# andabi/parallel-wavenet-vocoder

Measured on AMD Instinct MI355X. Metric: audio samples/sec, 4-flow IAF generation, higher is better.
Workload: dtype f32 via 3-term split-fp16 MFMA (fp32 accumulate, fp32 storage)

## Files before the change

### parallel-wavenet-vocoder_amd/csrc/pwv_layer_common.h

```cpp
#pragma once

#include "pwv_common.h"

namespace pwv {

constexpr int kA1 = 0;
constexpr int kA1Size = 4 * 16 * 64 * 4;
constexpr int kA2 = kA1 + kA1Size;
constexpr int kA2Size = 2 * 8 * 64 * 4;
constexpr int kBD = kA2 + kA2Size;
constexpr int kBDSize = 64;
constexpr int kLayerBase = kBD + kBDSize;
constexpr int kASSize = 4 * 8 * 64 * 4;
constexpr int kBSSize = 128;
constexpr int kCondC = 80;
constexpr int kACSize = 4 * (kCondC / 8) * 64 * 4;

constexpr int layer_floats(bool skip, bool cond) {
    return kLayerBase + (skip ? kASSize + kBSSize : 0) + (cond ? kACSize : 0);
}

constexpr int kHAS = 0;
constexpr int kHBS = kHAS + kASSize;
constexpr int kHA1 = kHBS + kBSSize;
constexpr int kHA1Size = 4 * 16 * 64 * 4;
constexpr int kHB1 = kHA1 + kHA1Size;
constexpr int kHW2 = kHB1 + 128;
constexpr int kMaxQ = 4;
constexpr int head_floats(int Q) { return kHW2 + 2 * Q * 64 + 4; }

struct LayerParams {
    const float* x_in[PWV_MAX_NETS];
    float* x_out[PWV_MAX_NETS];
    const float* packed[PWV_MAX_NETS];
    const float* proj[PWV_MAX_NETS];
    float* skip[PWV_MAX_NETS];
    const float* cond;
    int proj_row_stride;
    int G, N, T, dilation;
    int cond_hop, cond_offset, cond_frames;
    int skip_init;
    unsigned T_magic, T_shift;
    unsigned hop_magic, hop_shift;
    long long* trace;
    const float* x_first;
    const float* cfilt[PWV_MAX_NETS];
    const float* fold0[PWV_MAX_NETS];
    const float* packed_head[PWV_MAX_NETS];
    float* head_out[PWV_MAX_NETS];
    int head_q;
    float x_limit;
    int* range_flag;
};

struct StreamParams {
    const float* hist_rd;
    float* hist_wr;
    const int* slot_tab;
    long long block_stride;
    long long row_off[PWV_MAX_NETS];
    long long scalar_off;
};

inline void make_magic(unsigned d, unsigned& magic, unsigned& shift) {
    if (d <= 1) { magic = 0; shift = 0; return; }
    unsigned l = 0;
    while ((1ull << l) < d) ++l;
    const unsigned long long k = 31 + l;
    magic = (unsigned)(((1ull << k) + d - 1) / d);
    shift = l - 1;
}
__device__ __forceinline__ int fast_div(int n, unsigned magic, unsigned shift) {
    return magic ? (int)(__umulhi((unsigned)n, magic) >> shift) : n;
}

__device__ __forceinline__ void unit_rows(int unit, int lane, int rows, int N, int T, unsigned T_magic, unsigned T_shift,
                                          int& row, bool& valid, int& rc, int& n, int& t) {
    row = unit * 32 + (lane & 31);
    valid = row < rows;
    rc = valid ? row : rows - 1;
    if (T >= 32) {
        const int row0 = unit * 32;
        const int n0 = fast_div(row0, T_magic, T_shift);
        t = row0 - n0 * T + (lane & 31);
        n = n0;
        if (t >= T) { t -= T; n += 1; }
        if (!valid) { n = N - 1; t = T - 1; }
    } else {
        n = fast_div(rc, T_magic, T_shift);
        t = rc - n * T;
    }
}

constexpr int kVarlenRec = PWV_VARLEN_REC_INTS;
constexpr int kVarlenMinRows = 32;

__device__ __forceinline__ void unit_rows_varlen(const int* unit_map, int unit, int lane, int rows,
                                                 int& row, bool& valid, int& rc, int& fb, int& t) {
    typedef const __attribute__((address_space(4))) int* const_ints_t;
    row = unit * 32 + (lane & 31);
    valid = row < rows;
    rc = valid ? row : rows - 1;
    const int last = (rows - 1) >> 5;
    const const_ints_t rec = (const_ints_t)(unit_map + (size_t)(unit < last ? unit : last) * kVarlenRec);
    const int r0 = rec[1], f0 = rec[2], r1 = rec[3], f1 = rec[4];
    const bool second = rc >= r1;
    t = rc - (second ? r1 : r0);
    fb = second ? f1 : f0;
}

#ifdef PWV_TRACE
#define PWV_STAMP(slot)                                                                   \
    do {                                                                                  \
        if (p.trace && blockIdx.x < 2 && lane == 0 && tr_unit < 8)                        \
            p.trace[((blockIdx.x * 8 + wave) * 8 + tr_unit) * 16 + (slot)] = __builtin_amdgcn_s_memtime(); \
    } while (0)
#else
#define PWV_STAMP(slot) do {} while (0)
#endif

struct HeadParams {
    const float* in[PWV_MAX_NETS];
    const float* packed[PWV_MAX_NETS];
    float* out[PWV_MAX_NETS];
    int G, N, T, Q;
};

constexpr float kFScale = -2.8853900817779268f;
constexpr float kGScale = -1.4426950408889634f;
__device__ __forceinline__ float gate_act(float fs, float gs) {
#pragma clang fp contract(off)
    fs = __builtin_amdgcn_fmed3f(fs, -3.0e38f, 57.7f);
    gs = __builtin_amdgcn_fmed3f(gs, -3.0e38f, 57.7f);
    const float e1 = __builtin_amdgcn_exp2f(fs);
    const float e2 = __builtin_amdgcn_exp2f(gs);
    const float t = 1.f + e2;
    return (1.f - e1) * __builtin_amdgcn_rcpf(__builtin_fmaf(e1, t, t));
}

template <int N4, int THREADS>
__device__ __forceinline__ void fill_lds(float* lds, const float* __restrict__ packed, int tid) {
    constexpr int ITERS = (N4 + THREADS - 1) / THREADS;
    const f32x4* src = reinterpret_cast<const f32x4*>(packed);
    f32x4* dst = reinterpret_cast<f32x4*>(lds);
    f32x4 v[ITERS];
#pragma unroll
    for (int i = 0; i < ITERS; ++i) {
        const int idx = tid + i * THREADS;
        v[i] = src[idx < N4 ? idx : N4 - 1];
    }
#pragma unroll
    for (int i = 0; i < ITERS; ++i) {
        const int idx = tid + i * THREADS;
        if (idx < N4) dst[idx] = v[i];
    }
}

__host__ __device__ inline size_t tile32_floats(long long rows, int C) { return (size_t)((rows + 31) / 32) * 32 * C; }
__device__ __forceinline__ size_t tile_off(int row, int quad, int C) {
    return (size_t)(row >> 5) * (32 * C) + quad * 128 + (row & 31) * 4;
}
typedef unsigned u32x4 __attribute__((ext_vector_type(4)));
constexpr int kAuxWriteThrough = 16;
__device__ __forceinline__ __amdgpu_buffer_rsrc_t units_rsrc(const void* base, int u_begin, int u_end, int unit_bytes) {
    const unsigned long long a = (unsigned long long)base + (unsigned long long)u_begin * unit_bytes;
    const unsigned long long span = (unsigned long long)(u_end > u_begin ? u_end - u_begin : 0) * unit_bytes;
    const unsigned lo = __builtin_amdgcn_readfirstlane((unsigned)a), hi = __builtin_amdgcn_readfirstlane((unsigned)(a >> 32));
    const unsigned bytes = __builtin_amdgcn_readfirstlane((unsigned)(span > 0xffffffffull ? 0xffffffffull : span));
    return __builtin_amdgcn_make_buffer_rsrc((void*)(((unsigned long long)hi << 32) | lo), 0, bytes, 0x00020000);
}
__device__ __forceinline__ int units_off(int row, int quad, int C, int u_begin) {
    return (((row >> 5) - u_begin) * (32 * C) + quad * 128 + (row & 31) * 4) * 4;
}
template <typename V16>
__device__ __forceinline__ void store_wt(__amdgpu_buffer_rsrc_t r, int byte_off, V16 v) {
    static_assert(sizeof(V16) == 16, "store_wt moves 16 bytes");
    __builtin_amdgcn_raw_buffer_store_b128(__builtin_bit_cast(u32x4, v), r, byte_off, 0, kAuxWriteThrough);
}

typedef const __attribute__((address_space(1))) void* gptr_t;
typedef __attribute__((address_space(3))) void* lptr_t;
template <int N4, int WAVES>
__device__ __forceinline__ void fill_lds_dma(float* lds, const float* __restrict__ packed, int wave, int lane) {
    constexpr int CH = (N4 + 63) / 64;
#pragma unroll
    for (int i = 0; i < (CH + WAVES - 1) / WAVES; ++i) {
        const int c = wave + i * WAVES;
        if (c < CH && c * 64 + lane < N4)
            __builtin_amdgcn_global_load_lds((gptr_t)(packed + (size_t)(c * 64 + lane) * 4), (lptr_t)(lds + c * 256), 16, 0, 0);
    }
}

template <int NCH, int C>
__device__ __forceinline__ void load_tiled(const float* __restrict__ base, int row, int h, bool keep, float (&dst)[4 * NCH]) {
    const float* p0 = base + tile_off(row, h, C);
#pragma unroll
    for (int g = 0; g < NCH; ++g) {
        const f32x4 v = *reinterpret_cast<const f32x4*>(p0 + g * 256);
#pragma unroll
        for (int e = 0; e < 4; ++e) dst[4 * g + e] = keep ? v[e] : 0.f;
    }
}

template <int NCH>
__device__ __forceinline__ void load_row(const float* __restrict__ row, int h, bool keep, float (&dst)[4 * NCH]) {
#pragma unroll
    for (int g = 0; g < NCH; ++g) {
        const f32x4 v = *reinterpret_cast<const f32x4*>(row + 8 * g + 4 * h);
#pragma unroll
        for (int e = 0; e < 4; ++e) dst[4 * g + e] = keep ? v[e] : 0.f;
    }
}

template <int NCH>
__device__ __forceinline__ void load_contig(const float* __restrict__ p, float (&dst)[4 * NCH]) {
#pragma unroll
    for (int g = 0; g < NCH; ++g) {
        const f32x4 v = *reinterpret_cast<const f32x4*>(p + 4 * g);
#pragma unroll
        for (int e = 0; e < 4; ++e) dst[4 * g + e] = v[e];
    }
}


__device__ __forceinline__ f32x4 frag(const float* lds, int base, int it, int ngroups, int g, int lane) {
    return *reinterpret_cast<const f32x4*>(&lds[base + ((it * ngroups + g) * 64 + lane) * 4]);
}

template <int NG, int NIT, int IT0, int ITSTEP, int NACC, typename BF, typename EF, typename TF>
__device__ __forceinline__ void gemm_groups(const float* lds, int base, int lane, f32x16 (&acc)[NACC], f32x4 (&a)[4],
                                            BF&& bval, EF&& extra, TF&& tail) {
#pragma unroll
    for (int g = 0; g < NG; ++g) {
        f32x4 n[4] = {a[0], a[1], a[2], a[3]};
        if (g + 1 < NG) {
#pragma unroll
            for (int i = 0; i < NIT; ++i) n[i] = frag(lds, base, IT0 + i * ITSTEP, NG, g + 1, lane);
        } else {
            tail(n);
        }
        __builtin_amdgcn_sched_barrier(0);
#pragma unroll
        for (int e = 0; e < 4; ++e) {
            const float b = bval(g * 4 + e);
#pragma unroll
            for (int i = 0; i < NIT; ++i)
                acc[IT0 + i * ITSTEP] = __builtin_amdgcn_mfma_f32_32x32x2f32(a[i][e], b, acc[IT0 + i * ITSTEP], 0, 0, 0);
        }
        extra(g);
        __builtin_amdgcn_sched_barrier(0);
#pragma unroll
        for (int i = 0; i < 4; ++i) a[i] = n[i];
    }
}


int launch_stream_carry_ragged(const StreamParams& st, const int* tab, int n_carry, const int* cu_rows, int N, hipStream_t s);

int launch_layer_f16x3(const LayerParams& lp, bool skip, bool cond, bool gated, int per_net, hipStream_t s);
int launch_layer_f16x3_stream(const LayerParams& lp, const StreamParams& st, int per_net, hipStream_t s);
int launch_head_f16x3(const HeadParams& hp, bool from_gated, int grid, hipStream_t s);
int launch_pack_layer_f16x3(const float* filter, const float* gate, const float* dense, const float* dense_bias,
                            const float* skip, const float* skip_bias, const float* gc_filter, const float* gc_gate,
// ... 10 lines not shown
```

### parallel-wavenet-vocoder_amd/csrc/pwv_persist_exit.inc

```
    asm volatile("s_waitcnt vmcnt(0)" ::: "memory");
    if (!tail_done) {
        int old = 0;
        if (lane == 0) old = __hip_atomic_fetch_add(&ctl[4], 1, __ATOMIC_RELAXED, __HIP_MEMORY_SCOPE_WORKGROUP);
        if (__builtin_amdgcn_readfirstlane(old) == 7) {
            int done = 0;
            if (lane == 0) done = __hip_atomic_fetch_add(p.exited, 1, __ATOMIC_RELAXED, __HIP_MEMORY_SCOPE_AGENT);
            if (__builtin_amdgcn_readfirstlane(done) == p.active_wgs - 1) {
                for (int k = lane; k < p.G * p.nwg; k += 64) __hip_atomic_store(p.prog + (size_t)k * kProgStride, 0, __ATOMIC_RELAXED, __HIP_MEMORY_SCOPE_AGENT);
                if (SHORT) for (int k = lane; k < p.G * p.units; k += 64) __hip_atomic_store(p.uprog + (size_t)k * kUnitStride, 0, __ATOMIC_RELAXED, __HIP_MEMORY_SCOPE_AGENT);
                if (lane == 0) {
                    __hip_atomic_store(p.abort, 0, __ATOMIC_RELAXED, __HIP_MEMORY_SCOPE_AGENT);
                    __hip_atomic_store(p.exited, 0, __ATOMIC_RELAXED, __HIP_MEMORY_SCOPE_AGENT);
                }
            }
        }
    }
#ifdef PWV_PTRACE
    if (p.trace && lane == 0) {
        pt_acc[8] = __builtin_amdgcn_s_memtime();
        pt_acc[0] = pt_acc[8] - pt_start;
        long long* tr = p.trace + ((size_t)blockIdx.x * 8 + wave) * 24;
        for (int k = 0; k < 15; ++k) tr[k] = pt_acc[k];
        tr[16] = net; tr[17] = w; tr[18] = dead ? 1 : 0; tr[19] = __builtin_amdgcn_s_memrealtime(); tr[20] = pt_start_rt;
    }
#endif
```

### parallel-wavenet-vocoder_amd/csrc/pwv_persist_geometry.inc

```
    constexpr bool SHORT = MODE == 2;
    __shared__ __attribute__((aligned(16))) float lds[kLdsFloats];
    const int tid = threadIdx.x;
    const int lane = tid & 63;
    const int wave = __builtin_amdgcn_readfirstlane(tid >> 6);
    const int h = lane >> 5;

    int net, w;
    if (p.xcd_map) {
        const int x = blockIdx.x & 7, s = blockIdx.x >> 3;
        net = s % p.G;
        w = x * (p.nwg >> 3) + s / p.G;
    } else {
        net = blockIdx.x % p.G;
        w = blockIdx.x / p.G;
    }
    const int rows = p.N * p.T;
    auto rows_of = [&](int unit, int& row, bool& valid, int& rc, int& nn, int& t) {
        if constexpr (VARLEN) unit_rows_varlen(p.unit_map, unit, lane, rows, row, valid, rc, nn, t);
        else unit_rows(unit, lane, rows, p.N, p.T, p.T_magic, p.T_shift, row, valid, rc, nn, t);
    };
    auto p_base = [&](int nn) -> int {
        if constexpr (VARLEN) return nn;
        else return nn * p.cond_frames;
    };
    constexpr bool RAGGED = VARLEN && STREAM;
    auto unit_rec = [&](int unit, int& s0, int& r1) {
        typedef const __attribute__((address_space(4))) int* const_ints_t;
        const int last = (rows - 1) >> 5;
        const const_ints_t rec = (const_ints_t)(p.unit_map + (size_t)(unit < last ? unit : last) * kVarlenRec);
        s0 = rec[0];
        r1 = rec[3];
    };
    auto session_end = [&](int s0, int r1, bool second) -> int {
        return second ? p.cu_rows[s0 + 2] : r1;
    };
    (void)unit_rec;
    (void)session_end;
    const int u_begin = w * p.per_wg;
    const int u_end = u_begin + p.per_wg < p.units ? u_begin + p.per_wg : p.units;
    const int n = u_end - u_begin;
    if (n <= 0) return;
    const int L = p.n_layers;
    constexpr bool stat = SHORT;
    constexpr bool loader_mode = SHORT;
#ifdef PWV_PTRACE
    int pt_nev = 0;
#endif

    typedef __attribute__((address_space(3))) int* lds_ints_t;
    const lds_ints_t ctl = (lds_ints_t)(lds + kCtlF);
    typedef __attribute__((address_space(3))) volatile unsigned char* lds_bytes_t;
    const lds_bytes_t lb = (lds_bytes_t)lds;
    int* prog_n = p.prog + (size_t)net * p.nwg * kProgStride;
    int* uprog_n = p.uprog + (size_t)net * p.units * kUnitStride;
    const float* const proj_n = p.proj[net];
    const float* const packed_n = p.packed[net];
    const int v_dil = p.dil[lane & (kMaxPLayers - 1)];
    auto dil_of = [&](int j) -> int { return __builtin_amdgcn_readlane(v_dil, j); };
    auto dil_next = [&](int j) -> int { return j + 1 < L ? dil_of(j + 1) : (p.tail_q > 0 ? p.tail_dil : dil_of(j)); };

    for (int k = tid; k < (kLdsFloats - kCtlF); k += 512) ctl[k] = 0;
    __syncthreads();
    if (tid == 0) {
        lb[kSeenLB] = w > 0 ? 0 : 255;
        lb[kSeenRB] = w < p.last_wg ? 0 : 255;
        lb[kWreadyB] = 0;
        lb[kWreadyB + 1] = 1;
        lb[kTrueB] = 255;
    }
    auto fill_slot = [&](int slot, int layer, int first, int step) {
        const float* src = packed_n + (size_t)layer * p.packed_stride + lane * 4;
        float* dst = lds + slot * kSlot;
#pragma clang loop unroll(disable)
        for (int c = first; c < kSlot / 256; c += step)
            __builtin_amdgcn_global_load_lds((gptr_t)(src + c * 256), (lptr_t)(dst + c * 256), 16, 0, 0);
        if (first == 0 && lane < 16)
            __builtin_amdgcn_global_load_lds((gptr_t)(src + kSlotFull), (lptr_t)(lds + kBiasF + slot * 64), 16, 0, 0);
    };
    if (p.x_first && tid < 128) lds[kCfF + tid] = p.cfilt[net][tid];
    fill_slot(0, 0, wave, 8);
    if (L > 1) fill_slot(1, 1, wave, 8);
    __syncthreads();
    if (wave >= 4) __builtin_amdgcn_s_setprio(1);

    const __amdgpu_buffer_rsrc_t ring_rs = [&]() {
        const unsigned long long a = (unsigned long long)p.ring[net];
        const unsigned long long span = (unsigned long long)p.ring_stride * 8ull + (unsigned long long)p.units * 8192ull;
        const unsigned lo = __builtin_amdgcn_readfirstlane((unsigned)a), hi2 = __builtin_amdgcn_readfirstlane((unsigned)(a >> 32));
        return __builtin_amdgcn_make_buffer_rsrc((void*)(((unsigned long long)hi2 << 32) | lo), 0, __builtin_amdgcn_readfirstlane((unsigned)span), 0x00020000);
    }();
    const __amdgpu_buffer_rsrc_t proj_rs = [&]() {
        const unsigned long long a = (unsigned long long)proj_n;
        const unsigned lo = __builtin_amdgcn_readfirstlane((unsigned)a), hi2 = __builtin_amdgcn_readfirstlane((unsigned)(a >> 32));
        return __builtin_amdgcn_make_buffer_rsrc((void*)(((unsigned long long)hi2 << 32) | lo), 0, 0xFFFFFFFFu, 0x00020000);
    }();
    (void)proj_rs;
    const int slot_bytes = (int)(p.ring_stride * 4);
    int rot_pinned = 0;
    if constexpr (RAGGED) {
        rot_pinned = p.rot;
        asm volatile("" : "+s"(rot_pinned));
    }
    auto rot_of = [&]() -> int {
        if constexpr (RAGGED) return rot_pinned;
        else return p.rot;
    };
    auto in_soff = [&](int j) -> int { return ((j + 2 + rot_of()) % 3) * slot_bytes; };
    auto out_soff = [&](int j) -> int { return ((j + rot_of()) % 3) * slot_bytes; };
    auto toff = [&](int row) -> int { return ((row >> 5) * 2048 + h * 128 + (row & 31) * 4) * 4; };
    auto hist_lookback = [&](int jh, int d, int nn, int t, int unit, int rc, float (&xb)[32]) {
        if constexpr (STREAM) {
            if (!__all(t >= d)) {
                int sn = nn;
                if constexpr (RAGGED) {
                    int s0, r1, uu = unit;
                    asm volatile("" : "+s"(uu));
                    unit_rec(uu, s0, r1);
                    sn = s0 + (rc >= r1 ? 1 : 0);
                }
                if (t < d) {
                    const float* hr = p.hist_rd + (long long)p.slot_tab[2 * sn] * p.hist_block_stride + p.hist_off[net][jh] + tile_off(t, h, 64);
#pragma unroll
                    for (int g = 0; g < 8; ++g) {
                        const f32x4 v = *reinterpret_cast<const f32x4*>(hr + g * 256);
#pragma unroll
                        for (int e = 0; e < 4; ++e) xb[4 * g + e] = v[e];
                    }
                }
            }
        }
    };
    auto hist_store = [&](int jh, int d, int nn, int t, int unit, int rc, bool valid, const float (&xr)[32]) {
        if constexpr (RAGGED) {
            int s0, r1;
            unit_rec(unit, s0, r1);
            const bool second = rc >= r1;
            int k = rc + d - r1;
            if (__any(valid && (second || k >= 0))) {
                int lo = second ? 1 : 0;
                asm volatile("" : "+v"(lo));
                const int last = (rows - 1) >> 5;
                const int sn = p.unit_map[(size_t)(unit < last ? unit : last) * kVarlenRec] + lo;
                k = rc + d - p.cu_rows[sn + 1];
                if (valid && k >= 0) {
                    float* hw = p.hist_wr + (long long)p.slot_tab[2 * sn + 1] * p.hist_block_stride + p.hist_off[net][jh] + tile_off(k, h, 64);
#pragma unroll
                    for (int g = 0; g < 8; ++g) {
                        const f32x4 v = {xr[4 * g], xr[4 * g + 1], xr[4 * g + 2], xr[4 * g + 3]};
                        *reinterpret_cast<f32x4*>(hw + g * 256) = v;
                    }
                }
            }
        } else if constexpr (STREAM) {
            const int k = t + d - p.T;
            if (__any(valid && k >= 0)) {
                if (valid && k >= 0) {
                    float* hw = p.hist_wr + (long long)p.slot_tab[2 * nn + 1] * p.hist_block_stride + p.hist_off[net][jh] + tile_off(k, h, 64);
#pragma unroll
                    for (int g = 0; g < 8; ++g) {
                        const f32x4 v = {xr[4 * g], xr[4 * g + 1], xr[4 * g + 2], xr[4 * g + 3]};
                        *reinterpret_cast<f32x4*>(hw + g * 256) = v;
                    }
                }
            }
        }
    };

    auto load_x = [&](int j, int unit, float (&xb)[32], float (&xc)[32]) {
        int row, rc, nn, t;
        bool valid;
        rows_of(unit, row, valid, rc, nn, t);
        const int d = dil_of(j);
        const bool has_prev = t >= d;
        if (p.x_first && j == 0) {
            const float* x1 = p.x_first;
            xc[0] = x1[rc];
            xc[1] = t >= 1 ? x1[rc - (t >= 1 ? 1 : 0)] : 0.f;
            xb[0] = has_prev ? x1[rc - (has_prev ? d : 0)] : 0.f;
            xb[1] = t >= d + 1 ? x1[rc - (t >= d + 1 ? d + 1 : 0)] : 0.f;
#pragma unroll
            for (int k = 2; k < 32; ++k) xb[k] = xc[k] = 0.f;
            return;
        }
        const int so = in_soff(j);
        const int oc = toff(rc), ob = toff(has_prev ? rc - d : rc);
#pragma unroll
        for (int g = 0; g < 8; ++g) {
            const f32x4 v = __builtin_bit_cast(f32x4, __builtin_amdgcn_raw_buffer_load_b128(ring_rs, oc + g * 1024, so, 16));
#pragma unroll
            for (int e = 0; e < 4; ++e) xc[4 * g + e] = v[e];
        }
#pragma unroll
        for (int g = 0; g < 8; ++g) {
            const f32x4 v = __builtin_bit_cast(f32x4, __builtin_amdgcn_raw_buffer_load_b128(ring_rs, ob + g * 1024, so, 16));
#pragma unroll
            for (int e = 0; e < 4; ++e) xb[4 * g + e] = v[e];
        }
        if (!__all(has_prev)) {
#pragma unroll
            for (int k = 0; k < 32; ++k) xb[k] = has_prev ? xb[k] : 0.f;
        }
        hist_lookback(j, d, nn, t, unit, rc, xb);
    };

    auto load_xc = [&](int j, int unit, float (&xc)[32]) {
        int row, rc, nn, t;
        bool valid;
        rows_of(unit, row, valid, rc, nn, t);
        const int so = in_soff(j);
        const int oc = toff(rc);
#pragma unroll
        for (int g = 0; g < 8; ++g) {
            const f32x4 v = __builtin_bit_cast(f32x4, __builtin_amdgcn_raw_buffer_load_b128(ring_rs, oc + g * 1024, so, 16));
#pragma unroll
            for (int e = 0; e < 4; ++e) xc[4 * g + e] = v[e];
        }
    };
    auto load_xb = [&](int j, int unit, float (&xb)[32]) {
        int row, rc, nn, t;
        bool valid;
        rows_of(unit, row, valid, rc, nn, t);
        const int d = dil_of(j);
        const bool has_prev = t >= d;
        const int so = in_soff(j);
        const int ob = toff(has_prev ? rc - d : rc);
#pragma unroll
        for (int g = 0; g < 8; ++g) {
            const f32x4 v = __builtin_bit_cast(f32x4, __builtin_amdgcn_raw_buffer_load_b128(ring_rs, ob + g * 1024, so, 16));
#pragma unroll
            for (int e = 0; e < 4; ++e) xb[4 * g + e] = v[e];
        }
        hist_lookback(j, d, nn, t, unit, rc, xb);
    };
```

### parallel-wavenet-vocoder_amd/csrc/pwv_persist_tasks.inc

```
    if (u >= 0) {
        flush_owed();
        leave_layers(j);
        layer_vectors(j);
        if constexpr (SHORT) {
            load_xc(j, u, rxc);
        } else {
            const unsigned bad = eval(dep_addr(j, u));
            if (bad & kRawMask) wait_deps(j, u, kRawMask, j, 4);
            war_ok = (bad & kWarMask) == 0;
            if (!dead) load_x(j, u, rxb, rxc);
        }
    }
    int lv_j = j;

    while (u >= 0 && !dead) {
        PT_MARK();
        int row, rc, nn, t;
        bool valid;
        rows_of(u, row, valid, rc, nn, t);
        if constexpr (SHORT) {
            flush_owed();
            PT_EV(3, j, u);
            leave_layers(j);
        }
        f32x16 acc[4];
        if constexpr (SHORT) {
            int prow = 0;
            if (p.cond_hop > 0) prow = p_base(nn) + fast_div(t + p.cond_offset, p.hop_magic, p.hop_shift);
            const int po = (prow * p.proj_row_stride + j * 128 + h * 64) * 4;
#pragma unroll
            for (int it = 0; it < 4; ++it)
#pragma unroll
                for (int q = 0; q < 4; ++q) {
                    const f32x4 v = __builtin_bit_cast(f32x4, __builtin_amdgcn_raw_buffer_load_b128(proj_rs, po + (it * 16 + q * 4) * 4, 0, 0));
#pragma unroll
                    for (int e = 0; e < 4; ++e) acc[it][q * 4 + e] = v[e];
                }
        } else {
            int prow = 0;
            if (p.cond_hop > 0) prow = p_base(nn) + fast_div(t + p.cond_offset, p.hop_magic, p.hop_shift);
            const float* pr = proj_n + (size_t)prow * p.proj_row_stride + j * 128 + h * 64;
#pragma unroll
            for (int it = 0; it < 4; ++it)
#pragma unroll
                for (int q = 0; q < 4; ++q) {
                    const f32x4 v = *reinterpret_cast<const f32x4*>(pr + it * 16 + q * 4);
#pragma unroll
                    for (int e = 0; e < 4; ++e) acc[it][q * 4 + e] = v[e];
                }
        }
        if constexpr (SHORT) {
            PT_EV(15, j, u);
            if (lv_j != j) { layer_vectors(j); lv_j = j; }
            const unsigned bad = eval(dep_addr(j, u)) & ~1u;
            war_ok = (bad & kWarMask) == 0;
            if (bad & kRawMask) {
                wait_deps(j, u, kRawMask & ~1u, j, 4);
                if (dead) break;
            }
            PT_EV(16, j, u);
            load_xb(j, u, rxb);
            PT_EV(18, j, u);
        }
        int j2 = j;
        const int u2 = next_task(j, u, j2);
        unsigned bad2 = 0;
        if (u2 >= 0) {
            if (j2 != lv_j) { layer_vectors(j2); lv_j = j2; }
            bad2 = eval(dep_addr(j2, u2));
            if (stat) bad2 &= ~1u;
        }

        if (!SHORT && p.x_first && j == 0) {
            const float x0 = rxc[0], x1v = rxc[1], xd0 = rxb[0], xd1 = rxb[1];
            const bool has_prev = t >= dil_of(0);
            if (p.range_flag && !(fabsf(x0) <= p.x_limit)) __hip_atomic_store(p.range_flag, 1, __ATOMIC_RELAXED, __HIP_MEMORY_SCOPE_SYSTEM);
#pragma unroll
            for (int g = 0; g < 8; ++g) {
                const f32x4 w0 = *reinterpret_cast<const f32x4*>(&lds[kCfF + 8 * g + 4 * h]);
                const f32x4 w1 = *reinterpret_cast<const f32x4*>(&lds[kCfF + 64 + 8 * g + 4 * h]);
#pragma unroll
                for (int e = 0; e < 4; ++e) {
                    rxc[4 * g + e] = fmaf(x0, w1[e], x1v * w0[e]);
                    const float vb = fmaf(xd0, w1[e], xd1 * w0[e]);
                    rxb[4 * g + e] = has_prev ? vb : 0.f;
                }
            }
        }
        const float* bias = lds + kBiasF + (j & 1) * 64 + h * 32;
        float o[32];
        f32x16 acc2[2];
        auto settle_top = [&]() {
            PT_PHASE(9);
            if (!SHORT) PT_EV(5, j, u);
            PT_BEGIN();
            if (!SHORT) asm volatile("s_waitcnt vmcnt(0)" ::: "memory");
            PT_END(1);
            PT_EV(6, j, u);
            if constexpr (!SHORT) {
                publish();
                if (left_upto < j) leave_layers(j);
                if (u2 >= 0) claim_v = claim();
            }
            PT_ADD(5, 1);
            PT_MARK();
        };
        int early_v = -1;
        auto prefetch_next = [&]() {
            PT_PHASE(10);
            PT_BEGIN();
            if (u2 >= 0 && !(bad2 & kRawMask) && !stat) {
                load_x(j2, u2, rxb, rxc);
            } else {
#pragma unroll
                for (int k = 0; k < 32; ++k) rxb[k] = rxc[k] = 0.f;
            }
            if (stat && u2 >= 0 && (bad2 & 0x36u)) {
                const int a2 = dep_addr(j2, u2);
                const int cnt_r = w + p.reach_wgs < p.last_wg ? p.reach_wgs : p.last_wg - w;
                int lo = lane;
                asm volatile("" : "+v"(lo));
                if ((lo == 1 || lo == 2) && a2 >= kLeftB && a2 < kDoneB)
                    early_v = __hip_atomic_load(uprog_n + (size_t)(u_begin - kLeftN + a2 - kLeftB) * kUnitStride, __ATOMIC_RELAXED, __HIP_MEMORY_SCOPE_AGENT);
                else if ((bad2 & 0x30u) && lo >= 32 && lo - 32 < cnt_r)
                    early_v = __hip_atomic_load(prog_n + (size_t)(w + 1 + lo - 32) * kProgStride, __ATOMIC_RELAXED, __HIP_MEMORY_SCOPE_AGENT);
            }
            __builtin_amdgcn_sched_barrier(0);
            PT_LAP(13);
        };
        const float* lastfrag = packed_n + (size_t)j * p.packed_stride + kSlot + lane * 4;

        if constexpr (F32) {
#include "pwv_persist_unit_f32.inc"
        } else {
#include "pwv_persist_unit_f16x3.inc"
        }
        if (dead) break;
        PT_PHASE(11);
        PT_EV(1, j, u);
        if (!war_ok) {
            unsigned badw = kWarMask;
            if constexpr (SHORT) {
                if (lv_j != j) layer_vectors(j);
                badw = eval(dep_addr(j, u)) & kWarMask;
                if (lv_j != j) layer_vectors(lv_j);
            }
            if (badw) {
                PT_BEGIN();
                wait_deps(j, u, kWarMask, lv_j, 5);
                PT_END(3);
                if (dead) break;
            }
        }
        {
            const int so = out_soff(j);
            const int oo = toff(row);
            const int dn = dil_next(j);
            const bool shared = p.all_wt || u + ((dn + 31) >> 5) >= u_end;
            if (valid) {
                if (shared) {
#pragma unroll
                    for (int g = 0; g < 8; ++g) {
                        const int it = g >> 2, q = g & 3;
                        const f32x4 v = {acc2[it][q * 4], acc2[it][q * 4 + 1], acc2[it][q * 4 + 2], acc2[it][q * 4 + 3]};
                        __builtin_amdgcn_raw_buffer_store_b128(__builtin_bit_cast(u32x4, v), ring_rs, oo + g * 1024, so, kAuxWriteThrough);
                    }
                } else {
#pragma unroll
                    for (int g = 0; g < 8; ++g) {
                        const int it = g >> 2, q = g & 3;
                        const f32x4 v = {acc2[it][q * 4], acc2[it][q * 4 + 1], acc2[it][q * 4 + 2], acc2[it][q * 4 + 3]};
                        __builtin_amdgcn_raw_buffer_store_b128(__builtin_bit_cast(u32x4, v), ring_rs, oo + g * 1024, so, kStoreAuxLocal);
                    }
                }
            }
        }
        __builtin_amdgcn_sched_barrier(0);
        PT_EV(2, j, u);

        prev_addr = kDoneB + (u - u_begin);
        prev_j = j;
        if (stat && u2 >= 0 && (bad2 & 0x36u)) {
            const int a2 = dep_addr(j2, u2);
            if (early_v >= 0 && lane < 32) lb[a2] = (unsigned char)(early_v > 255 ? 255 : early_v);
            if ((bad2 & 0x30u) && w < p.last_wg && __ballot(lane >= 32 && early_v >= 0 && early_v < j2 - 1) == 0 && (int)lb[kSeenRB] < j2 - 1)
                lb[kSeenRB] = (unsigned char)(j2 - 1);
        }
        if constexpr (SHORT) {
#pragma unroll
            for (int k = 0; k < 32; ++k) rxc[k] = acc2[k >> 4][k & 15];
        } else if (u2 >= 0 && (bad2 & kRawMask)) {
            PT_BEGIN();
            PT_ADD(6, 1);
            wait_deps(j2, u2, kRawMask, lv_j, 4);
            PT_END(2);
            if (dead) break;
            load_x(j2, u2, rxb, rxc);
        }
        j = j2;
        u = u2;
        if constexpr (!SHORT) war_ok = (bad2 & kWarMask) == 0;
        PT_PHASE(12);
    }
    asm volatile("s_waitcnt vmcnt(0)" ::: "memory");
    if (!dead && !(loader_mode && wave >= n)) {
        publish();
        leave_layers(L);
        if (dma_pending >= 0) flush_owed();
    }
```

### parallel-wavenet-vocoder_amd/csrc/pwv_persist_unit_f16x3.inc

```
            const f16x8* A1 = reinterpret_cast<const f16x8*>(lds + (j & 1) * kSlot);
            const f16x8* A2 = reinterpret_cast<const f16x8*>(lds + (j & 1) * kSlot + kA1Size);

            f16x8 bh[8], bl[8];
            float xc[32];
#pragma unroll
            for (int k = 0; k < 32; ++k) xc[k] = rxc[k];
            split8<0>(xc, bh[4], bl[4]);
            split8<8>(xc, bh[5], bl[5]);
            split8<16>(xc, bh[6], bl[6]);
            split8<24>(xc, bh[7], bl[7]);
            settle_top();
            hist_store(j, dil_of(j), nn, t, u, rc, valid, xc);
            auto bxh = [&](int s) -> f16x8 { return bh[s ^ 4]; };
            auto bxl = [&](int s) -> f16x8 { return bl[s ^ 4]; };
            f16x8 oh[4], ol[4];
            f16x8 ah[4], al[4];
            f16x8 lf = {0, 0, 0, 0, 0, 0, 0, 0};

            {
            first_frags<8, 2, 0, 2, 4>(A1, lane, ah, al);
            gemm16<8, 2, 0, 2, 4>(
                A1, lane, acc, ah, al, bxh, bxl,
                [&](int s) {
                    if constexpr (SHORT) {
                        if (s == 3) {
                            PT_EV(14, j, u);
                            if constexpr (!STREAM) {
                                if (!__all(t >= dil_of(j))) {
                                    const bool hp = t >= dil_of(j);
#pragma unroll
                                    for (int k = 0; k < 32; ++k) rxb[k] = hp ? rxb[k] : 0.f;
                                }
                            }
                            split8<0>(rxb, bh[0], bl[0]);
                            split8<8>(rxb, bh[1], bl[1]);
                            split8<16>(rxb, bh[2], bl[2]);
                            split8<24>(rxb, bh[3], bl[3]);
                            asm volatile("" : "+v"(bh[0]), "+v"(bl[0]), "+v"(bh[1]), "+v"(bl[1]), "+v"(bh[2]), "+v"(bl[2]), "+v"(bh[3]), "+v"(bl[3]));
                            PT_EV(5, j, u);
                        }
                    } else {
                        if (s == 0) { split8<0>(rxb, bh[0], bl[0]); asm volatile("" : "+v"(bh[0]), "+v"(bl[0])); }
                        if (s == 1) { split8<8>(rxb, bh[1], bl[1]); asm volatile("" : "+v"(bh[1]), "+v"(bl[1])); }
                        if (s == 2) { split8<16>(rxb, bh[2], bl[2]); asm volatile("" : "+v"(bh[2]), "+v"(bl[2])); }
                        if (s == 3) { split8<24>(rxb, bh[3], bl[3]); asm volatile("" : "+v"(bh[3]), "+v"(bl[3])); }
                    }
                },
                [&](f16x8(&nh)[4], f16x8(&nl)[4]) { first_frags<8, 2, 1, 2, 4>(A1, lane, nh, nl); });
            gemm16<8, 2, 1, 2, 4>(
                A1, lane, acc, ah, al, bxh, bxl,
                [&](int s) {
                    o[2 * s] = gate_act(acc[0][2 * s], acc[2][2 * s]);
                    o[2 * s + 1] = gate_act(acc[0][2 * s + 1], acc[2][2 * s + 1]);
                    asm volatile("" : "+v"(o[2 * s]), "+v"(o[2 * s + 1]));
                    if (s == 3) { split8<0>(o, oh[0], ol[0]); asm volatile("" : "+v"(oh[0]), "+v"(ol[0])); }
                    if (s == 7) { split8<8>(o, oh[1], ol[1]); asm volatile("" : "+v"(oh[1]), "+v"(ol[1])); }
                    if (s == 5) lf = *reinterpret_cast<const f16x8*>(lastfrag);
                },
                [&](f16x8(&nh)[4], f16x8(&nl)[4]) { first_frags<4, 2, 0, 1, 2>(A2, lane, nh, nl); });
            }

#pragma unroll
            for (int it = 0; it < 2; ++it)
#pragma unroll
                for (int q = 0; q < 4; ++q) {
                    const f32x4 bd = *reinterpret_cast<const f32x4*>(bias + it * 16 + q * 4);
#pragma unroll
                    for (int e = 0; e < 4; ++e) acc2[it][q * 4 + e] = xc[it * 16 + q * 4 + e] + bd[e];
                }
            asm volatile("" : "+v"(acc2[0]), "+v"(acc2[1]), "+v"(lf));
            prefetch_next();
            gemm16_dense(
                [&](int comp, int it, int s) -> f16x8 { return (comp == 1 && it == 1 && s == 3) ? lf : frag16<4, 2>(A2, comp, it, s, lane); },
                acc2, ah, al, [&](int s) -> f16x8 { return oh[s]; }, [&](int s) -> f16x8 { return ol[s]; },
                [&](int s) {
                    if (s < 2) {
#pragma unroll
                        for (int e = 0; e < 8; ++e) o[16 + 8 * s + e] = gate_act(acc[1][8 * s + e], acc[3][8 * s + e]);
                        if (s == 0) split8<16>(o, oh[2], ol[2]);
                        else split8<24>(o, oh[3], ol[3]);
                        asm volatile("" : "+v"(oh[2 + (s & 1)]), "+v"(ol[2 + (s & 1)]));
                    }
                });
            PT_LAP(14);
```

### parallel-wavenet-vocoder_amd/csrc/pwv_persist_unit_f32.inc

```
            float xc[32], xb[32];
#pragma unroll
            for (int k = 0; k < 32; ++k) { xc[k] = rxc[k]; xb[k] = rxb[k]; }
            if constexpr (SHORT && !STREAM) {
                if (!__all(t >= dil_of(j))) {
                    const bool hp = t >= dil_of(j);
#pragma unroll
                    for (int k = 0; k < 32; ++k) xb[k] = hp ? xb[k] : 0.f;
                }
            }
            settle_top();
            hist_store(j, dil_of(j), nn, t, u, rc, valid, xc);
            const float* Af = lds + (j & 1) * kSlot;
            f32x4 a[4];
            f32x4 lf = {0.f, 0.f, 0.f, 0.f};
            auto bx = [&](int ks) -> float { return ks < 32 ? xb[ks] : xc[ks - 32]; };
            a[0] = frag(Af, 0, 0, 16, 0, lane);
            a[1] = frag(Af, 0, 2, 16, 0, lane);
            gemm_groups<16, 2, 0, 2>(Af, 0, lane, acc, a, bx, [](int) {}, [&](f32x4(&nf)[4]) {
                nf[0] = frag(Af, 0, 1, 16, 0, lane);
                nf[1] = frag(Af, 0, 3, 16, 0, lane);
            });
            gemm_groups<16, 2, 1, 2>(
                Af, 0, lane, acc, a, bx,
                [&](int g) {
                    o[g] = gate_act(acc[0][g], acc[2][g]);
                    asm volatile("" : "+v"(o[g]));
                    if (g == 10) lf = *reinterpret_cast<const f32x4*>(lastfrag);
                },
                [&](f32x4(&nf)[4]) {
                    nf[0] = frag(Af, kA1Size, 0, 8, 0, lane);
                    nf[1] = frag(Af, kA1Size, 1, 8, 0, lane);
                });
#pragma unroll
            for (int it = 0; it < 2; ++it)
#pragma unroll
                for (int q = 0; q < 4; ++q) {
                    const f32x4 bd = *reinterpret_cast<const f32x4*>(bias + it * 16 + q * 4);
#pragma unroll
                    for (int e = 0; e < 4; ++e) acc2[it][q * 4 + e] = xc[it * 16 + q * 4 + e] + bd[e];
                }
            asm volatile("" : "+v"(acc2[0]), "+v"(acc2[1]), "+v"(lf));
            prefetch_next();
            gemm_groups_dense(
                [&](int it, int g) -> f32x4 { return (it == 1 && g == 7) ? lf : frag(Af, kA1Size, it, 8, g, lane); }, acc2, a,
                [&](int ks) -> float { return o[ks]; },
                [&](int g) {
                    if (g < 4) {
#pragma unroll
                        for (int e = 0; e < 4; ++e) {
                            o[16 + 4 * g + e] = gate_act(acc[1][4 * g + e], acc[3][4 * g + e]);
                            asm volatile("" : "+v"(o[16 + 4 * g + e]));
                        }
                    }
                });
            PT_LAP(14);
```

### parallel-wavenet-vocoder_amd/csrc/pwv_stack_persist.hip

```cpp
#include "pwv_f16x3.h"
#include "pwv_persist_plan.h"

#include <cstddef>
#include <cstdlib>
#include <cstring>

namespace pwv {

constexpr int kStoreAuxLocal = 0;

constexpr int kSlotFull = kA1Size + kA2Size;
constexpr int kSlot = kSlotFull - 256;
constexpr int kBiasF = 2 * kSlot;
constexpr int kCtlF = kBiasF + 128;
constexpr int kCtlInts = 40;
constexpr int kLdsFloats = 40960;
constexpr int kCfF = kCtlF + kCtlInts;
constexpr int kLeftB = (kCfF + 128) * 4;
constexpr int kDoneB = kLeftB + kLeftN;
constexpr int kMaxUnitsWgLds = kLdsFloats * 4 - kDoneB;
static_assert(kMaxUnitsWg == kMaxUnitsWgLds && kPlanMaxQ == kMaxQ, "pwv_persist_plan.h restates the kernel's limits");
static_assert(kUnitModeMaxPerWg <= 7, "the short-input instantiation keeps wave 7 as its loader");
static_assert(kLeftN <= 32, "unit mode: the right neighbours are polled by lanes 32..63 alone");
constexpr int kFlagB = (kCtlF + 2) * 4;
constexpr int kSeenLB = kFlagB, kSeenRB = kFlagB + 1, kWreadyB = kFlagB + 2, kTrueB = kFlagB + 4;
constexpr long long kWaitTicks = 2000000;

struct PersistParams {
    float* ring[PWV_MAX_NETS];
    long long ring_stride;
    const float* packed[PWV_MAX_NETS];
    const float* proj[PWV_MAX_NETS];
    int* prog;
    int* uprog;
    int unit_mode;
    int* abort;
    int* exited;
    int active_wgs;
    int* status;
    long long packed_stride;
    int proj_row_stride;
    int G, N, T, n_layers, units, per_wg, nwg, last_wg, reach_wgs, xcd_map, rot;
    int all_wt;
    int cond_hop, cond_offset, cond_frames;
    unsigned T_magic, T_shift, hop_magic, hop_shift;
    int dil[kMaxPLayers];
    const float* x_first;
    const float* cfilt[PWV_MAX_NETS];
    const float* fold0[PWV_MAX_NETS];
    float x_limit;
    int* range_flag;
    long long* trace;
    long long* trace_ev;
    const float* tail_layer[PWV_MAX_NETS];
    const float* tail_head[PWV_MAX_NETS];
    float* tail_out[PWV_MAX_NETS];
    int tail_q, tail_dil, tail_reach_wgs;
    const float* affine_x;
    float* affine_out;
    int* pair;
    const int* unit_map;
    const float* hist_rd;
    float* hist_wr;
    const int* slot_tab;
    long long hist_block_stride;
    long long hist_scalar_off;
    long long hist_off[PWV_MAX_NETS][kMaxPLayers + 1];
    const int* cu_rows;
};

#ifdef PWV_PTRACE
#define PT_DECL long long pt_acc[15] = {0, 0, 0, 0, 0, 0, 0, 0, 0, 0, 0, 0, 0, 0, 0}; long long pt_t = 0, pt_p = 0; (void)pt_t; (void)pt_p;
#define PT_BEGIN() pt_t = __builtin_amdgcn_s_memtime()
#define PT_END(k) pt_acc[k] += __builtin_amdgcn_s_memtime() - pt_t
#define PT_ADD(k, v) pt_acc[k] += (v)
#define PT_LAP(k) do { __builtin_amdgcn_sched_barrier(0); const long long pt_n = __builtin_amdgcn_s_memtime(); pt_acc[k] += pt_n - pt_t; pt_t = pt_n; __builtin_amdgcn_sched_barrier(0); } while (0)
#define PT_MARK() do { __builtin_amdgcn_sched_barrier(0); pt_p = __builtin_amdgcn_s_memtime(); __builtin_amdgcn_sched_barrier(0); } while (0)
#define PT_PHASE(k) do { __builtin_amdgcn_sched_barrier(0); const long long pt_n = __builtin_amdgcn_s_memtime(); pt_acc[k] += pt_n - pt_p; pt_p = pt_n; __builtin_amdgcn_sched_barrier(0); } while (0)
#define PT_EV(code, jj, uu) do { if (p.trace_ev && pt_nev < 64) { if (lane == 0) { long long* e_ = p.trace_ev + (((size_t)blockIdx.x * 8 + wave) * 64 + pt_nev) * 4; \
    e_[0] = __builtin_amdgcn_s_memrealtime(); e_[1] = (code); e_[2] = (jj); e_[3] = (long long)(uu); } ++pt_nev; } } while (0)
#else
#define PT_DECL
#define PT_BEGIN() do {} while (0)
#define PT_END(k) do {} while (0)
#define PT_ADD(k, v) do {} while (0)
#define PT_LAP(k) do {} while (0)
#define PT_MARK() do {} while (0)
#define PT_PHASE(k) do {} while (0)
#define PT_EV(code, jj, uu) do {} while (0)
#endif

constexpr unsigned kRawMask = 0xFu, kWarMask = 0x30u;

template <typename FR, typename BH, typename BL, typename EF>
__device__ __forceinline__ void gemm16_dense(FR&& fr, f32x16 (&acc)[2], f16x8 (&ah)[4], f16x8 (&al)[4], BH&& bh, BL&& bl, EF&& extra) {
#pragma unroll
    for (int s = 0; s < 4; ++s) {
        f16x8 nh[2] = {ah[0], ah[1]};
        f16x8 nl[2] = {al[0], al[1]};
        if (s + 1 < 4) {
#pragma unroll
            for (int i = 0; i < 2; ++i) {
                nh[i] = fr(0, i, s + 1);
                nl[i] = fr(1, i, s + 1);
            }
        }
        __builtin_amdgcn_sched_barrier(0);
        const f16x8 b_h = bh(s);
        const f16x8 b_l = bl(s);
#pragma unroll
        for (int i = 0; i < 2; ++i) acc[i] = __builtin_amdgcn_mfma_f32_32x32x16_f16(ah[i], b_h, acc[i], 0, 0, 0);
#pragma unroll
        for (int i = 0; i < 2; ++i) acc[i] = __builtin_amdgcn_mfma_f32_32x32x16_f16(ah[i], b_l, acc[i], 0, 0, 0);
#pragma unroll
        for (int i = 0; i < 2; ++i) acc[i] = __builtin_amdgcn_mfma_f32_32x32x16_f16(al[i], b_h, acc[i], 0, 0, 0);
        extra(s);
        __builtin_amdgcn_sched_barrier(0);
#pragma unroll
        for (int i = 0; i < 2; ++i) {
            ah[i] = nh[i];
            al[i] = nl[i];
        }
    }
}

template <typename FR, typename BF, typename EF>
__device__ __forceinline__ void gemm_groups_dense(FR&& fr, f32x16 (&acc)[2], f32x4 (&a)[4], BF&& bval, EF&& extra) {
#pragma unroll
    for (int g = 0; g < 8; ++g) {
        f32x4 n[2] = {a[0], a[1]};
        if (g + 1 < 8) {
#pragma unroll
            for (int i = 0; i < 2; ++i) n[i] = fr(i, g + 1);
        }
        __builtin_amdgcn_sched_barrier(0);
#pragma unroll
        for (int e = 0; e < 4; ++e) {
            const float b = bval(g * 4 + e);
#pragma unroll
            for (int i = 0; i < 2; ++i) acc[i] = __builtin_amdgcn_mfma_f32_32x32x2f32(a[i][e], b, acc[i], 0, 0, 0);
        }
        extra(g);
        __builtin_amdgcn_sched_barrier(0);
#pragma unroll
        for (int i = 0; i < 2; ++i) a[i] = n[i];
    }
}

template <bool F32, int MODE, bool VARLEN, bool STREAM = false>
__global__ __launch_bounds__(512) void stack_persist_kernel(const PersistParams p) {
    static_assert(!(VARLEN && STREAM), "streaming of packed batches is not built");
#include "pwv_stack_persist_body.inc"
}

template <bool F32, int MODE>
__global__ __launch_bounds__(512) void stack_persist_ragged_kernel(const PersistParams p) {
    constexpr bool VARLEN = true, STREAM = true;
#include "pwv_stack_persist_body.inc"
}

__global__ __launch_bounds__(256) void stream_carry_ragged_kernel(const StreamParams st, const int* __restrict__ tab, const int* __restrict__ cu_rows) {
    const int e = blockIdx.x, n = blockIdx.y;
    const int T = cu_rows[n + 1] - cu_rows[n];
    const int off = tab[4 * e], len = tab[4 * e + 1], width = tab[4 * e + 2];
    const int keep = len - T;
    if (keep <= 0) return;
    const int2 blk = reinterpret_cast<const int2*>(st.slot_tab)[n];
    const float* src = st.hist_rd + (long long)blk.x * st.block_stride + off;
    float* dst = st.hist_wr + (long long)blk.y * st.block_stride + off;
    if (width == 1) {
        for (int k = threadIdx.x; k < keep; k += blockDim.x) dst[k] = src[k + T];
        return;
    }
    const int total = ((keep + 31) >> 5) * 512;
    for (int i = threadIdx.x; i < total; i += blockDim.x) {
        const int k = (i >> 9) * 32 + (i & 31), q = (i >> 5) & 15;
        if (k < keep) *reinterpret_cast<f32x4*>(dst + tile_off(k, q, 64)) = *reinterpret_cast<const f32x4*>(src + tile_off(k + T, q, 64));
    }
}

int launch_stream_carry_ragged(const StreamParams& st, const int* tab, int n_carry, const int* cu_rows, int N, hipStream_t s) {
    hipLaunchKernelGGL(stream_carry_ragged_kernel, dim3(n_carry, N), dim3(256), 0, s, st, tab, cu_rows);
    PWV_CHECK_HIP(hipGetLastError());
    return PWV_OK;
}

__global__ void persist_zero_kernel(int4* p, size_t n16) {
    const size_t i = (size_t)blockIdx.x * blockDim.x + threadIdx.x;
    if (i < n16) p[i] = int4{0, 0, 0, 0};
}

__global__ void varlen_unit_map_kernel(const int* __restrict__ cu_rows, const int* __restrict__ cu_frames, int n_utt, int units, int* __restrict__ out) {
    const int u = blockIdx.x * blockDim.x + threadIdx.x;
    if (u >= units) return;
    const int r = u * 32;
    int lo = 0, hi = n_utt - 1;
    while (lo < hi) {
        const int mid = (lo + hi + 1) >> 1;
        if (cu_rows[mid] <= r) lo = mid;
        else hi = mid - 1;
    }
    int4* o = reinterpret_cast<int4*>(out + (size_t)u * kVarlenRec);
    o[0] = int4{lo, cu_rows[lo], cu_frames ? cu_frames[lo] : 0, cu_rows[lo + 1]};
    o[1] = int4{cu_frames ? cu_frames[lo + 1] : 0, 0, 0, 0};
}

}

using namespace pwv;

extern "C" {

int pwv_persist_status(int** status) {
    static int* g_status = nullptr;
    PWV_CHECK_ARG(status, "pwv_persist_status: NULL argument");
    if (!g_status) {
        PWV_CHECK_HIP(hipHostMalloc((void**)&g_status, sizeof(int), hipHostMallocMapped | hipHostMallocPortable));
        *g_status = 0;
    }
    *status = g_status;
    return PWV_OK;
}

#ifndef RAGGED_F32
#define RAGGED_F32 1
// ... 240 lines not shown
```

Measured before the change: 60.37 million.

## Use buffer loads and lane-packed scalars for the per-unit projection and weight fetches

Packs the projection stride, hop divisor constants, cond offset and cond frames into spare lanes of the dilation VGPR, read with readlane, so the non-short path avoids scalar kernel-argument loads. Projection rows and weight-slot fills now go through buffer resource loads with a wave-uniform base and per-lane offsets, replacing flat global loads. The varlen unit record is loaded once per unit and reused by the history store. Finer waitcnt placement and register pinning are added around the split, along with extra trace counters. Together these aim to cut address arithmetic and scalar-load latency on the layer's critical path, at the cost of more subtle memory ordering to get right.

Result: faster. 61.28 million (median of 6 runs) (+1.5%).

```diff
diff --git a/parallel-wavenet-vocoder_amd/csrc/pwv_layer_common.h b/parallel-wavenet-vocoder_amd/csrc/pwv_layer_common.h
--- a/parallel-wavenet-vocoder_amd/csrc/pwv_layer_common.h
+++ b/parallel-wavenet-vocoder_amd/csrc/pwv_layer_common.h
@@ -109,6 +109,24 @@
     fb = second ? f1 : f0;
 }
 
+__device__ __forceinline__ void unit_record_varlen(const int* unit_map, int unit, int rows, int (&rec)[4]) {
+    typedef const __attribute__((address_space(4))) int* const_ints_t;
+    const int last = (rows - 1) >> 5;
+    const const_ints_t r = (const_ints_t)(unit_map + (size_t)(unit < last ? unit : last) * kVarlenRec);
+    rec[0] = r[1];
+    rec[1] = r[2];
+    rec[2] = r[3];
+    rec[3] = r[4];
+}
+__device__ __forceinline__ void unit_rows_from_record(const int (&rec)[4], int unit, int lane, int rows, int& row, bool& valid, int& rc, int& fb, int& t) {
+    row = unit * 32 + (lane & 31);
+    valid = row < rows;
+    rc = valid ? row : rows - 1;
+    const bool second = rc >= rec[2];
+    t = rc - (second ? rec[2] : rec[0]);
+    fb = second ? rec[3] : rec[1];
+}
+
 #ifdef PWV_TRACE
 #define PWV_STAMP(slot)                                                                   \
     do {                                                                                  \
diff --git a/parallel-wavenet-vocoder_amd/csrc/pwv_persist_exit.inc b/parallel-wavenet-vocoder_amd/csrc/pwv_persist_exit.inc
--- a/parallel-wavenet-vocoder_amd/csrc/pwv_persist_exit.inc
+++ b/parallel-wavenet-vocoder_amd/csrc/pwv_persist_exit.inc
@@ -21,6 +21,7 @@
         pt_acc[0] = pt_acc[8] - pt_start;
         long long* tr = p.trace + ((size_t)blockIdx.x * 8 + wave) * 24;
         for (int k = 0; k < 15; ++k) tr[k] = pt_acc[k];
+        for (int k = 15; k < 18; ++k) tr[k + 6] = pt_acc[k];
         tr[16] = net; tr[17] = w; tr[18] = dead ? 1 : 0; tr[19] = __builtin_amdgcn_s_memrealtime(); tr[20] = pt_start_rt;
     }
 #endif
diff --git a/parallel-wavenet-vocoder_amd/csrc/pwv_persist_geometry.inc b/parallel-wavenet-vocoder_amd/csrc/pwv_persist_geometry.inc
--- a/parallel-wavenet-vocoder_amd/csrc/pwv_persist_geometry.inc
+++ b/parallel-wavenet-vocoder_amd/csrc/pwv_persist_geometry.inc
@@ -19,9 +19,22 @@
         if constexpr (VARLEN) unit_rows_varlen(p.unit_map, unit, lane, rows, row, valid, rc, nn, t);
         else unit_rows(unit, lane, rows, p.N, p.T, p.T_magic, p.T_shift, row, valid, rc, nn, t);
     };
+    constexpr int kLaneStride = kMaxPLayers, kLaneHopMagic = kMaxPLayers + 1, kLaneHopShift = kMaxPLayers + 2, kLaneCondOffset = kMaxPLayers + 3,
+                  kLaneCondFrames = kMaxPLayers + 4;
+    static_assert(kMaxPLayers + 5 <= 64, "the dilations and the P row's scalars share one VGPR");
+    int v_dil = p.dil[lane & (kMaxPLayers - 1)];
+    if constexpr (!SHORT) {
+        const int k = lane - kMaxPLayers;
+        const int c = k == 0 ? p.proj_row_stride : (k == 1 ? (int)p.hop_magic : (k == 2 ? (int)p.hop_shift : (k == 3 ? p.cond_offset : p.cond_frames)));
+        v_dil = k >= 0 ? c : v_dil;
+    }
+    auto dil_of = [&](int j) -> int { return __builtin_amdgcn_readlane(v_dil, j); };
+    auto top_scalar = [&](int k) -> int { return __builtin_amdgcn_readlane(v_dil, k); };
+    (void)top_scalar;
     auto p_base = [&](int nn) -> int {
         if constexpr (VARLEN) return nn;
-        else return nn * p.cond_frames;
+        else if constexpr (SHORT) return nn * p.cond_frames;
+        else return nn * top_scalar(kLaneCondFrames);
     };
     constexpr bool RAGGED = VARLEN && STREAM;
     auto unit_rec = [&](int unit, int& s0, int& r1) {
@@ -55,8 +68,6 @@
     int* uprog_n = p.uprog + (size_t)net * p.units * kUnitStride;
     const float* const proj_n = p.proj[net];
     const float* const packed_n = p.packed[net];
-    const int v_dil = p.dil[lane & (kMaxPLayers - 1)];
-    auto dil_of = [&](int j) -> int { return __builtin_amdgcn_readlane(v_dil, j); };
     auto dil_next = [&](int j) -> int { return j + 1 < L ? dil_of(j + 1) : (p.tail_q > 0 ? p.tail_dil : dil_of(j)); };
 
     for (int k = tid; k < (kLdsFloats - kCtlF); k += 512) ctl[k] = 0;
@@ -71,6 +82,14 @@
     auto fill_slot = [&](int slot, int layer, int first, int step) {
         const float* src = packed_n + (size_t)layer * p.packed_stride + lane * 4;
         float* dst = lds + slot * kSlot;
+        if constexpr (!SHORT) {
+            const __amdgpu_buffer_rsrc_t prs = __builtin_amdgcn_make_buffer_rsrc((void*)(packed_n + (size_t)layer * p.packed_stride), 0, (kSlotFull + 64) * 4, 0x00020000);
+#pragma clang loop unroll(disable)
+            for (int c = first; c < kSlot / 256; c += step)
+                __builtin_amdgcn_raw_ptr_buffer_load_lds(prs, (lptr_t)(dst + c * 256), 16, lane * 16, c * 1024, 0, 0);
+            if (first == 0 && lane < 16) __builtin_amdgcn_raw_ptr_buffer_load_lds(prs, (lptr_t)(lds + kBiasF + slot * 64), 16, lane * 16, kSlotFull * 4, 0, 0);
+            return;
+        }
 #pragma clang loop unroll(disable)
         for (int c = first; c < kSlot / 256; c += step)
             __builtin_amdgcn_global_load_lds((gptr_t)(src + c * 256), (lptr_t)(dst + c * 256), 16, 0, 0);
@@ -95,6 +114,10 @@
         return __builtin_amdgcn_make_buffer_rsrc((void*)(((unsigned long long)hi2 << 32) | lo), 0, 0xFFFFFFFFu, 0x00020000);
     }();
     (void)proj_rs;
+    auto proj_rs_at = [&](long long floats) -> __amdgpu_buffer_rsrc_t {
+        return __builtin_amdgcn_make_buffer_rsrc((void*)(proj_n + floats), 0, 0xFFFFFFFFu, 0x00020000);
+    };
+    (void)proj_rs_at;
     const int slot_bytes = (int)(p.ring_stride * 4);
     int rot_pinned = 0;
     if constexpr (RAGGED) {
@@ -130,10 +153,11 @@
             }
         }
     };
-    auto hist_store = [&](int jh, int d, int nn, int t, int unit, int rc, bool valid, const float (&xr)[32]) {
+    auto hist_store = [&](int jh, int d, int nn, int t, int unit, int rc, bool valid, const float (&xr)[32], int r1_top = -1) {
         if constexpr (RAGGED) {
-            int s0, r1;
-            unit_rec(unit, s0, r1);
+            int s0 = 0, r1 = r1_top;
+            if (r1_top < 0) unit_rec(unit, s0, r1);
+            (void)s0;
             const bool second = rc >= r1;
             int k = rc + d - r1;
             if (__any(valid && (second || k >= 0))) {
@@ -166,10 +190,21 @@
         }
     };
 
+    int top_rec[4] = {0, 0, 0, 0};
+    auto rows_of_top = [&](int unit, int& row, bool& valid, int& rc, int& nn, int& t) {
+        if constexpr (VARLEN && !SHORT) unit_rows_from_record(top_rec, unit, lane, rows, row, valid, rc, nn, t);
+        else rows_of(unit, row, valid, rc, nn, t);
+    };
+    (void)rows_of_top;
     auto load_x = [&](int j, int unit, float (&xb)[32], float (&xc)[32]) {
         int row, rc, nn, t;
         bool valid;
-        rows_of(unit, row, valid, rc, nn, t);
+        if constexpr (VARLEN && !SHORT) {
+            unit_record_varlen(p.unit_map, unit, rows, top_rec);
+            unit_rows_from_record(top_rec, unit, lane, rows, row, valid, rc, nn, t);
+        } else {
+            rows_of(unit, row, valid, rc, nn, t);
+        }
         const int d = dil_of(j);
         const bool has_prev = t >= d;
         if (p.x_first && j == 0) {
diff --git a/parallel-wavenet-vocoder_amd/csrc/pwv_persist_tasks.inc b/parallel-wavenet-vocoder_amd/csrc/pwv_persist_tasks.inc
--- a/parallel-wavenet-vocoder_amd/csrc/pwv_persist_tasks.inc
+++ b/parallel-wavenet-vocoder_amd/csrc/pwv_persist_tasks.inc
@@ -15,9 +15,10 @@
 
     while (u >= 0 && !dead) {
         PT_MARK();
+        PT_BEGIN();
         int row, rc, nn, t;
         bool valid;
-        rows_of(u, row, valid, rc, nn, t);
+        rows_of_top(u, row, valid, rc, nn, t);
         if constexpr (SHORT) {
             flush_owed();
             PT_EV(3, j, u);
@@ -38,16 +39,20 @@
                 }
         } else {
             int prow = 0;
-            if (p.cond_hop > 0) prow = p_base(nn) + fast_div(t + p.cond_offset, p.hop_magic, p.hop_shift);
-            const float* pr = proj_n + (size_t)prow * p.proj_row_stride + j * 128 + h * 64;
+            if (p.cond_hop > 0) prow = p_base(nn) + fast_div(t + top_scalar(kLaneCondOffset), (unsigned)top_scalar(kLaneHopMagic), (unsigned)top_scalar(kLaneHopShift));
+            const int stride = top_scalar(kLaneStride);
+            const int prow0 = __builtin_amdgcn_readfirstlane(prow);
+            const __amdgpu_buffer_rsrc_t prs = proj_rs_at((long long)prow0 * stride);
+            const int po = ((prow - prow0) * stride + h * 64) * 4;
 #pragma unroll
             for (int it = 0; it < 4; ++it)
 #pragma unroll
                 for (int q = 0; q < 4; ++q) {
-                    const f32x4 v = *reinterpret_cast<const f32x4*>(pr + it * 16 + q * 4);
+                    const f32x4 v = __builtin_bit_cast(f32x4, __builtin_amdgcn_raw_buffer_load_b128(prs, po + (it * 16 + q * 4) * 4, j * 512, 0));
 #pragma unroll
                     for (int e = 0; e < 4; ++e) acc[it][q * 4 + e] = v[e];
                 }
+            PT_LAP(15);
         }
         if constexpr (SHORT) {
             PT_EV(15, j, u);
@@ -86,6 +91,10 @@
                     rxb[4 * g + e] = has_prev ? vb : 0.f;
                 }
             }
+            const float n0 = rxc[0], n1 = rxc[1], m0 = rxb[0], m1 = rxb[1];
+            __builtin_amdgcn_sched_barrier(0);
+            asm volatile("v_mov_b32 %0, %4\n\tv_mov_b32 %1, %5\n\tv_mov_b32 %2, %6\n\tv_mov_b32 %3, %7"
+                         : "=&v"(rxc[0]), "=&v"(rxc[1]), "=&v"(rxb[0]), "=&v"(rxb[1]) : "v"(n0), "v"(n1), "v"(m0), "v"(m1));
         }
         const float* bias = lds + kBiasF + (j & 1) * 64 + h * 32;
         float o[32];
@@ -95,6 +104,7 @@
             if (!SHORT) PT_EV(5, j, u);
             PT_BEGIN();
             if (!SHORT) asm volatile("s_waitcnt vmcnt(0)" ::: "memory");
+            if (!SHORT) __builtin_amdgcn_s_waitcnt(0x0F70);
             PT_END(1);
             PT_EV(6, j, u);
             if constexpr (!SHORT) {
diff --git a/parallel-wavenet-vocoder_amd/csrc/pwv_persist_unit_f16x3.inc b/parallel-wavenet-vocoder_amd/csrc/pwv_persist_unit_f16x3.inc
--- a/parallel-wavenet-vocoder_amd/csrc/pwv_persist_unit_f16x3.inc
+++ b/parallel-wavenet-vocoder_amd/csrc/pwv_persist_unit_f16x3.inc
@@ -3,14 +3,19 @@
 
             f16x8 bh[8], bl[8];
             float xc[32];
+            if constexpr (!SHORT) __builtin_amdgcn_s_waitcnt(0x4F70);
 #pragma unroll
             for (int k = 0; k < 32; ++k) xc[k] = rxc[k];
             split8<0>(xc, bh[4], bl[4]);
+            if constexpr (!SHORT) PT_LAP(16);
             split8<8>(xc, bh[5], bl[5]);
             split8<16>(xc, bh[6], bl[6]);
             split8<24>(xc, bh[7], bl[7]);
+            if constexpr (!SHORT)
+                asm volatile("" : "+v"(bh[4]), "+v"(bl[4]), "+v"(bh[5]), "+v"(bl[5]), "+v"(bh[6]), "+v"(bl[6]), "+v"(bh[7]), "+v"(bl[7]));
+            if constexpr (!SHORT) PT_LAP(17);
             settle_top();
-            hist_store(j, dil_of(j), nn, t, u, rc, valid, xc);
+            hist_store(j, dil_of(j), nn, t, u, rc, valid, xc, (RAGGED && !SHORT) ? top_rec[2] : -1);
             auto bxh = [&](int s) -> f16x8 { return bh[s ^ 4]; };
             auto bxl = [&](int s) -> f16x8 { return bl[s ^ 4]; };
             f16x8 oh[4], ol[4];
diff --git a/parallel-wavenet-vocoder_amd/csrc/pwv_persist_unit_f32.inc b/parallel-wavenet-vocoder_amd/csrc/pwv_persist_unit_f32.inc
--- a/parallel-wavenet-vocoder_amd/csrc/pwv_persist_unit_f32.inc
+++ b/parallel-wavenet-vocoder_amd/csrc/pwv_persist_unit_f32.inc
@@ -9,7 +9,7 @@
                 }
             }
             settle_top();
-            hist_store(j, dil_of(j), nn, t, u, rc, valid, xc);
+            hist_store(j, dil_of(j), nn, t, u, rc, valid, xc, (RAGGED && !SHORT) ? top_rec[2] : -1);
             const float* Af = lds + (j & 1) * kSlot;
             f32x4 a[4];
             f32x4 lf = {0.f, 0.f, 0.f, 0.f};
diff --git a/parallel-wavenet-vocoder_amd/csrc/pwv_stack_persist.hip b/parallel-wavenet-vocoder_amd/csrc/pwv_stack_persist.hip
--- a/parallel-wavenet-vocoder_amd/csrc/pwv_stack_persist.hip
+++ b/parallel-wavenet-vocoder_amd/csrc/pwv_stack_persist.hip
@@ -70,7 +70,7 @@
 };
 
 #ifdef PWV_PTRACE
-#define PT_DECL long long pt_acc[15] = {0, 0, 0, 0, 0, 0, 0, 0, 0, 0, 0, 0, 0, 0, 0}; long long pt_t = 0, pt_p = 0; (void)pt_t; (void)pt_p;
+#define PT_DECL long long pt_acc[18] = {0, 0, 0, 0, 0, 0, 0, 0, 0, 0, 0, 0, 0, 0, 0, 0, 0, 0}; long long pt_t = 0, pt_p = 0; (void)pt_t; (void)pt_p;
 #define PT_BEGIN() pt_t = __builtin_amdgcn_s_memtime()
 #define PT_END(k) pt_acc[k] += __builtin_amdgcn_s_memtime() - pt_t
 #define PT_ADD(k, v) pt_acc[k] += (v)
```
